# Arief-AK/OpenCL-Development-Real-time-Image-Processing

Measured on AMD Instinct MI355X. Metric: Mpixels/s (Gaussian 5x5, 4K RGBA), higher is better.
Workload: dtype u8 in/out, f32 accumulate

## Files before the change

### opencl-development-real-time-image-processing_amd/csrc/capi.hip

```cpp
#include <hip/hip_runtime.h>

#include <cmath>
#include <cstdio>
#include <cstdlib>
#include <cstring>
#include <ctime>
#include <new>
#include <vector>

#include "../../include/mi355_imgfilter.h"
#include "kernels.hpp"

using namespace mi355;

namespace {

struct CoefEntry {
    int k;
    uint32_t sigma_bits;
    GaussCoef coef;
    float* d_buf;
    std::vector<float> h_tab;
    uint64_t last_use;
    bool installed;
};

constexpr size_t kMaxCoefEntries = 16;
constexpr size_t kMaxInstalledCoefs = 64;

struct DevBuf {
    void* p;
    size_t cap;
};

}

struct mi355_ctx {
    int device = 0;
    hipStream_t stream = nullptr;
    bool own_stream = false;
    hipEvent_t ev[6] = {};
    hipEvent_t t0 = nullptr, t1 = nullptr;
    DevBuf d_in = {}, d_out = {};
    DevBuf d_raw = {};
    DevBuf d_flags = {};
    DevBuf d_hist = {};
    DevBuf d_lut = {};
    DevBuf d_ccl = {};
    DevBuf d_map1 = {}, d_map2 = {};
    unsigned long long* d_acc = nullptr;
    float* d_img_table = nullptr;
    static constexpr int kSlots = 3;
    hipStream_t s_h2d = nullptr, s_d2h = nullptr;
    hipEvent_t ev_h2d[kSlots] = {}, ev_k[kSlots] = {}, ev_d2h[kSlots] = {};
    DevBuf slot_in[kSlots] = {}, slot_out[kSlots] = {}, slot_raw[kSlots] = {};
    int input_format = MI355_INPUT_RGBA;
    int gauss_mode = MI355_GAUSS_FAST;
    int impl = MI355_IMPL_AUTO;
    int last_hip = 0;
    char name[256] = {};
    std::vector<CoefEntry> coefs;
    uint64_t coef_clock = 0;
    std::vector<void*> pinned;
};

namespace {

#define HIP_TRY(ctx, expr)                     \
    do {                                       \
        hipError_t e__ = (expr);               \
        if (e__ != hipSuccess) {               \
            if (ctx)                           \
                (ctx)->last_hip = (int)e__;    \
            return MI355_ERR_HIP;              \
        }                                      \
    } while (0)

uint64_t now_ns()
{
    timespec ts;
    clock_gettime(CLOCK_MONOTONIC, &ts);
    return (uint64_t)ts.tv_sec * 1000000000ull + (uint64_t)ts.tv_nsec;
}

uint32_t fbits(float f)
{
    uint32_t u;
    std::memcpy(&u, &f, 4);
    return u;
}

bool valid_k(int k) { return k >= 1 && k <= MI355_MAX_GAUSS_K && (k & 1) == 1; }
bool valid_sigma(float s) { return std::isfinite(s) && s > 0.0f; }

void gen_weights(int k, float sigma, float* out)
{
    const int half = k / 2;
    float sum = 0.0f;
    for (int y = -half; y <= half; y++) {
        for (int x = -half; x <= half; x++) {
            const float arg = -(x * x + y * y) / (2 * sigma * sigma);
            const float value = (float)(std::exp((double)arg) / (2 * M_PI * sigma * sigma));
            out[(y + half) * k + (x + half)] = value;
            sum += value;
        }
    }
    for (int i = 0; i < k * k; i++)
        out[i] /= sum;
}

void gen_weights_image2d(int k, float sigma, float* out)
{
    const int half = k / 2;
    for (int i = 0; i < k * k; i++)
        out[i] = 0.0f;
    float sum = 0.0f;
    for (int x = -half; x < half; x++) {
        for (int y = -half; y < half; y++) {
            const float arg = -((x * x + y * y) / (2 * sigma * sigma));
            const float value = (float)(std::exp((double)arg) / (2 * M_PI * sigma * sigma));
            out[(x + half) * k + (y + half)] = value;
// ... 7 lines not shown
bool separable_factor(int k, const float* w2d, float* w1d)
{
    double tot = 0.0, wmax = 0.0;
    bool nonneg = true;
    std::vector<double> rs(k, 0.0);
    for (int i = 0; i < k; i++) {
        for (int j = 0; j < k; j++) {
            const double v = (double)w2d[i * k + j];
            rs[i] += v;
            nonneg = nonneg && v >= 0.0;
            wmax = std::fmax(wmax, std::fabs(v));
        }
        tot += rs[i];
    }
    if (!nonneg || !(tot > 0.0)) {
        for (int i = 0; i < k; i++)
            w1d[i] = 0.0f;
        return false;
    }
    const double s = std::sqrt(tot);
    for (int i = 0; i < k; i++)
        w1d[i] = (float)(rs[i] / s);
    double dev = 0.0;
    for (int i = 0; i < k; i++)
        for (int j = 0; j < k; j++)
            dev = std::fmax(dev, std::fabs((double)w2d[i * k + j] - (double)w1d[i] * (double)w1d[j]));
    return dev <= 1.0e-6 * wmax;
}

int install_coef(mi355_ctx* ctx, int k, float sigma, const float* w2d, bool installed, const GaussCoef** out)
{
    CoefEntry* slot = nullptr;
    size_t n_generated = 0, n_installed = 0;
    for (auto& e : ctx->coefs) {
        if (e.k == k && e.sigma_bits == fbits(sigma))
            slot = &e;
        (e.installed ? n_installed : n_generated)++;
    }
    if (!slot) {
        if (installed && n_installed >= kMaxInstalledCoefs)
            return MI355_ERR_BAD_ARG;
        if (!installed && n_generated >= kMaxCoefEntries) {
            HIP_TRY(ctx, hipStreamSynchronize(ctx->stream));
            size_t lru = ctx->coefs.size();
            for (size_t i = 0; i < ctx->coefs.size(); i++)
                if (!ctx->coefs[i].installed && (lru == ctx->coefs.size() || ctx->coefs[i].last_use < ctx->coefs[lru].last_use))
                    lru = i;
            (void)hipFree(ctx->coefs[lru].d_buf);
            ctx->coefs.erase(ctx->coefs.begin() + (long)lru);
        }
        CoefEntry e{};
        e.k = k;
        e.sigma_bits = fbits(sigma);
        HIP_TRY(ctx, hipMalloc((void**)&e.d_buf, sizeof(float) * (size_t)(k * k + k + 512)));
        ctx->coefs.push_back(e);
        slot = &ctx->coefs.back();
    }
    slot->last_use = ++ctx->coef_clock;
    slot->installed = slot->installed || installed;
    std::vector<float> host((size_t)k * k + k + 512);
    std::memcpy(host.data(), w2d, sizeof(float) * (size_t)k * k);
    const bool separable = separable_factor(k, w2d, host.data() + (size_t)k * k);
    uint32_t alpha_tab[256];
    for (uint32_t a = 0; a < 256; a++)
        alpha_tab[a] = gauss_const_alpha(host.data() + (size_t)k * k, k, a) << 24;
    std::memcpy(host.data() + (size_t)k * k + k, alpha_tab, sizeof(alpha_tab));
    uint32_t alpha_cpu[256];
    for (uint32_t a = 0; a < 256; a++) {
        float chain = 0.0f;
        for (int i = 0; i < k * k; i++)
            chain += (float)a * w2d[i];
        chain = chain < 0.0f ? 0.0f : (chain > 255.0f ? 255.0f : chain);
        alpha_cpu[a] = (uint32_t)chain << 16;
    }
    std::memcpy(host.data() + (size_t)k * k + k + 256, alpha_cpu, sizeof(alpha_cpu));
    const hipError_t ce = hipMemcpy(slot->d_buf, host.data(), sizeof(float) * host.size(), hipMemcpyHostToDevice);
    if (ce != hipSuccess) {
        ctx->last_hip = (int)ce;
        (void)hipFree(slot->d_buf);
        ctx->coefs.erase(ctx->coefs.begin() + (slot - ctx->coefs.data()));
        return MI355_ERR_HIP;
    }
    slot->coef.k = k;
    slot->coef.separable = separable;
    slot->coef.d_w2d = slot->d_buf;
    slot->coef.d_w1d = slot->d_buf + (size_t)k * k;
    slot->coef.d_alpha_tab = reinterpret_cast<const uint32_t*>(slot->d_buf + (size_t)k * k + k);
    std::memcpy(slot->coef.h_alpha_tab, alpha_tab, sizeof(alpha_tab));
    slot->coef.d_alpha_cpu = reinterpret_cast<const uint32_t*>(slot->d_buf + (size_t)k * k + k + 256);
    std::memcpy(slot->coef.h_alpha_cpu, alpha_cpu, sizeof(alpha_cpu));
    std::memset(slot->coef.h_w1d, 0, sizeof(slot->coef.h_w1d));
    std::memcpy(slot->coef.h_w1d, host.data() + (size_t)k * k, sizeof(float) * k);
    slot->h_tab = host;
    slot->coef.h_w2d = slot->h_tab.data();
    if (out)
        *out = &slot->coef;
    return MI355_OK;
}

int get_coef(mi355_ctx* ctx, int k, float sigma, const GaussCoef** out)
{
    for (auto& e : ctx->coefs)
        if (e.k == k && e.sigma_bits == fbits(sigma)) {
            e.last_use = ++ctx->coef_clock;
            *out = &e.coef;
            return MI355_OK;
        }
    std::vector<float> w((size_t)k * k);
    gen_weights(k, sigma, w.data());
    return install_coef(ctx, k, sigma, w.data(), false, out);
}

int ensure(mi355_ctx* ctx, DevBuf& b, size_t need)
{
    if (b.cap >= need)
        return MI355_OK;
    if (b.p) {
        HIP_TRY(ctx, hipStreamSynchronize(ctx->stream));
        HIP_TRY(ctx, hipFree(b.p));
        b = {};
    }
    size_t want = need + need / 4;
    hipError_t e = hipMalloc(&b.p, want);
    if (e != hipSuccess) {
        e = hipMalloc(&b.p, need);
        want = need;
    }
    if (e != hipSuccess) {
        ctx->last_hip = (int)e;
        b.p = nullptr;
        return MI355_ERR_NOMEM;
    }
    b.cap = want;
    return MI355_OK;
}

int ensure_slots(mi355_ctx* ctx, DevBuf (&slots)[mi355_ctx::kSlots], size_t need)
{
    if (slots[0].cap >= need)
        return MI355_OK;
    HIP_TRY(ctx, hipDeviceSynchronize());
    for (DevBuf& b : slots) {
        if (b.p)
            (void)hipFree(b.p);
        b = {};
    }
    for (DevBuf& b : slots)
        if (hipMalloc(&b.p, need) != hipSuccess)
            return MI355_ERR_NOMEM;
    for (DevBuf& b : slots)
        b.cap = need;
    return MI355_OK;
}

enum class KRule { none, gauss, median, morph, box };

struct FilterInfo {
    int id;
    int in_bpp, out_bpp;
    KRule k;
    bool table;
    bool below_2g;
};

constexpr FilterInfo kFilters[] = {
    {MI355_FILTER_GRAY, 4, 4, KRule::none, false, false},
// ... 337 lines not shown
    if (!(rx < limit) || !(ry < limit))
        return MI355_ERR_UNSUPPORTED;
    if (inv)
        for (int k = 0; k < 6; k++)
            inv[k] = i[k];
    return MI355_OK;
}

int check_two_shapes(int bpp, int src_w, int src_h, int dst_w, int dst_h, int nframes, int border_mode)
{
    if (bad_shapes(bpp, src_w, src_h, dst_w, dst_h, nframes, border_mode))
        return MI355_ERR_BAD_ARG;
    const int rc = check_shape_limits(src_w, src_h, dst_w, dst_h, nframes);
    if (rc == MI355_OK && remap_work_items(dst_w, dst_h, nframes) > 0x7FFFFFF0ull)
        return MI355_ERR_BAD_ARG;
    return rc;
}

void map_bytes(int dst_w, int dst_h, int map_kind, size_t* n1, size_t* n2)
{
    const size_t entries = (size_t)dst_w * dst_h;
    *n1 = entries * 4;
    *n2 = entries * (map_kind == MI355_MAP_FIXED ? 2 : 4);
}

void perspective_inverse(const double m[9], int flags, double inv[9])
{
    if (flags & MI355_WARP_INVERSE_MAP) {
        for (int i = 0; i < 9; i++)
            inv[i] = m[i];
        return;
    }
    const double det = m[0] * (m[4] * m[8] - m[5] * m[7]) - m[1] * (m[3] * m[8] - m[5] * m[6]) +
                       m[2] * (m[3] * m[7] - m[4] * m[6]);
    const double d = (det != 0.0) ? 1.0 / det : 0.0;
    inv[0] = (m[4] * m[8] - m[5] * m[7]) * d;
    inv[1] = (m[2] * m[7] - m[1] * m[8]) * d;
    inv[2] = (m[1] * m[5] - m[2] * m[4]) * d;
    inv[3] = (m[5] * m[6] - m[3] * m[8]) * d;
    inv[4] = (m[0] * m[8] - m[2] * m[6]) * d;
    inv[5] = (m[2] * m[3] - m[0] * m[5]) * d;
    inv[6] = (m[3] * m[7] - m[4] * m[6]) * d;
    inv[7] = (m[1] * m[6] - m[0] * m[7]) * d;
    inv[8] = (m[0] * m[4] - m[1] * m[3]) * d;
}

int check_perspective(int bpp, int src_w, int src_h, int dst_w, int dst_h, int nframes, const double* m, int flags,
                      int border_mode, double* inv)
{
    if (!m || !warp_flags_ok(flags) || bad_shapes(bpp, src_w, src_h, dst_w, dst_h, nframes, border_mode) ||
        !all_finite(m, 9))
        return MI355_ERR_BAD_ARG;
    const int rc = check_two_shapes(bpp, src_w, src_h, dst_w, dst_h, nframes, border_mode);
    if (rc == MI355_OK && inv)
        perspective_inverse(m, flags, inv);
    return rc;
}

int adaptive_idelta(int type, double delta)
{
    const double d = type == MI355_ADAPTIVE_BINARY ? std::ceil(delta) : std::floor(delta);
    return d < -256.0 ? -256 : (d > 256.0 ? 256 : (int)d);
}

int create_common(int device, hipStream_t stream, bool own, mi355_ctx** out)
{
    if (!out)
        return MI355_ERR_BAD_ARG;
    *out = nullptr;
    int n = 0;
    if (hipGetDeviceCount(&n) != hipSuccess || n <= 0)
        return MI355_ERR_NO_DEVICE;
    if (device < 0 || device >= n)
        return MI355_ERR_NO_DEVICE;
    hipDeviceProp_t prop;
    if (hipGetDeviceProperties(&prop, device) != hipSuccess)
        return MI355_ERR_NO_DEVICE;
    if (std::strncmp(prop.gcnArchName, "gfx950", 6) != 0)
        return MI355_ERR_UNSUPPORTED;
    mi355_ctx* ctx = new (std::nothrow) mi355_ctx();
    if (!ctx)
        return MI355_ERR_NOMEM;
    ctx->device = device;
    std::snprintf(ctx->name, sizeof(ctx->name), "%s (%s)", prop.name, prop.gcnArchName);
    bool ok = hipSetDevice(device) == hipSuccess;
    if (ok && own)
        ok = hipStreamCreateWithFlags(&stream, hipStreamNonBlocking) == hipSuccess;
    ctx->stream = stream;
    ctx->own_stream = own && ok;
    for (int i = 0; ok && i < 6; i++)
        ok = hipEventCreate(&ctx->ev[i]) == hipSuccess;
    ok = ok && hipEventCreate(&ctx->t0) == hipSuccess && hipEventCreate(&ctx->t1) == hipSuccess;
    ok = ok && hipMalloc((void**)&ctx->d_acc, sizeof(unsigned long long)) == hipSuccess;
    if (!ok) {
        mi355_ctx_destroy(ctx);
        return MI355_ERR_HIP;
    }
    *out = ctx;
    return MI355_OK;
}

}

extern "C" {

#define MI355_API __attribute__((visibility("default")))

MI355_API int mi355_device_count(int* count)
{
    if (!count)
        return MI355_ERR_BAD_ARG;
    int n = 0;
    if (hipGetDeviceCount(&n) != hipSuccess)
        n = 0;
    *count = n;
    return MI355_OK;
}

MI355_API int mi355_ctx_create(int device, mi355_ctx** out)
{
    return create_common(device, nullptr, true, out);
}

MI355_API int mi355_ctx_create_on_stream(int device, void* hip_stream, mi355_ctx** out)
{
    return create_common(device, static_cast<hipStream_t>(hip_stream), false, out);
}

MI355_API int mi355_ctx_destroy(mi355_ctx* ctx)
{
    if (!ctx)
        return MI355_ERR_BAD_ARG;
    (void)hipSetDevice(ctx->device);
    (void)hipStreamSynchronize(ctx->stream);
    for (auto& e : ctx->coefs)
        (void)hipFree(e.d_buf);
    for (void* p : ctx->pinned)
        (void)hipHostFree(p);
    for (void* p : {(void*)ctx->d_acc, (void*)ctx->d_img_table, ctx->d_in.p, ctx->d_out.p, ctx->d_raw.p, ctx->d_flags.p,
                    ctx->d_hist.p, ctx->d_lut.p, ctx->d_ccl.p, ctx->d_map1.p, ctx->d_map2.p})
        if (p)
            (void)hipFree(p);
    for (int i = 0; i < mi355_ctx::kSlots; i++) {
        for (void* p : {ctx->slot_in[i].p, ctx->slot_out[i].p, ctx->slot_raw[i].p})
            if (p)
                (void)hipFree(p);
        for (hipEvent_t ev : {ctx->ev_h2d[i], ctx->ev_k[i], ctx->ev_d2h[i]})
            if (ev)
                (void)hipEventDestroy(ev);
    }
    for (hipStream_t s : {ctx->s_h2d, ctx->s_d2h})
        if (s)
            (void)hipStreamDestroy(s);
    for (hipEvent_t ev : {ctx->ev[0], ctx->ev[1], ctx->ev[2], ctx->ev[3], ctx->ev[4], ctx->ev[5], ctx->t0, ctx->t1})
        if (ev)
            (void)hipEventDestroy(ev);
    if (ctx->own_stream && ctx->stream)
        (void)hipStreamDestroy(ctx->stream);
    delete ctx;
    return MI355_OK;
}

MI355_API int mi355_ctx_device_name(mi355_ctx* ctx, char* buf, size_t buflen)
{
    if (!ctx || !buf || buflen == 0)
        return MI355_ERR_BAD_ARG;
// ... 1234 lines not shown
```

### opencl-development-real-time-image-processing_amd/csrc/common.hpp

```cpp
#pragma once
#include <hip/hip_runtime.h>
#include <stdint.h>

#include <cstdlib>
#include <type_traits>
#include <utility>

namespace mi355 {

constexpr int kWave = 64;

template <int... Ks, typename F>
hipError_t dispatch_int(int v, std::integer_sequence<int, Ks...>, F&& f)
{
    hipError_t e = hipErrorInvalidValue;
    (void)((v == Ks && ((e = f(std::integral_constant<int, Ks>{})), true)) || ...);
    return e;
}

template <typename F>
hipError_t dispatch_bool(bool v, F&& f)
{
    return v ? f(std::true_type{}) : f(std::false_type{});
}

inline bool aligned_to(const void* p, size_t n)
{
    return (reinterpret_cast<uintptr_t>(p) & (n - 1)) == 0;
}

inline bool rows_ragged(int w, const void* d_in, size_t in_align, const void* d_out, size_t out_align)
{
    return (w & 3) != 0 || !aligned_to(d_in, in_align) || !aligned_to(d_out, out_align);
}

inline bool gauss_upper_clamp(double wsum, double slack = 0.0)
{
    return !(255.0 * wsum * wsum * 1.0001 + slack < 256.0);
}

inline const char* tune_env(const char* name)
{
#ifdef MI355_TUNE_ENV
    return getenv(name);
#else
    (void)name;
    return nullptr;
#endif
}

using u32x4 = __attribute__((ext_vector_type(4))) uint32_t;
using u32x2 = __attribute__((ext_vector_type(2))) uint32_t;
using f32x4 = __attribute__((ext_vector_type(4))) float;

__device__ __forceinline__ uint32_t luma_rgb(uint32_t r, uint32_t g, uint32_t b)
{
    double v = 0.299 * (double)r + 0.587 * (double)g + 0.114 * (double)b;
    return (uint32_t)v;
}

__device__ __forceinline__ uint32_t luma_px(uint32_t px)
{
    return luma_rgb(px & 0xFFu, (px >> 8) & 0xFFu, (px >> 16) & 0xFFu);
}

__device__ __forceinline__ float luma_px_fast(uint32_t px)
{
    const uint32_t hi = __builtin_amdgcn_udot4(px, 0x00000201u, 0u, false);
    const uint32_t lo = __builtin_amdgcn_udot4(px, 0x00724B2Bu, 0u, false);
    const float S = (float)((hi << 8) + lo);
    float q = __builtin_floorf(__builtin_fmaf(S, 0.001f, 0.0005f));
    if (__builtin_fmaf(q, -1000.0f, S) == 0.0f)
        q = (float)luma_px(px);
    return q;
}

__device__ __forceinline__ void fill_gray_lut(uint8_t* gray_lut)
{
    gray_lut[threadIdx.x] = (uint8_t)luma_rgb(threadIdx.x, threadIdx.x, threadIdx.x);
}

__device__ __forceinline__ uint32_t luma_px_ambiguous(uint32_t px, const uint8_t* gray_lut)
{
    if (((px ^ (px >> 8)) & 0xFFFFu) == 0u)
        return gray_lut[px & 0xFFu];
    return luma_px(px);
}

__device__ __forceinline__ void luma_quad_fast(const u32x4& p, float g[4])
{
    float rem[4];
#pragma unroll
    for (int j = 0; j < 4; j++) {
        const uint32_t hi = __builtin_amdgcn_udot4(p[j], 0x00000201u, 0u, false);
        const uint32_t lo = __builtin_amdgcn_udot4(p[j], 0x00724B2Bu, 0u, false);
        const float S = (float)((hi << 8) + lo);
        g[j] = __builtin_floorf(__builtin_fmaf(S, 0.001f, 0.0005f));
        rem[j] = __builtin_fmaf(g[j], -1000.0f, S);
    }
    if (fminf(fminf(rem[0], rem[1]), fminf(rem[2], rem[3])) == 0.0f) {
#pragma unroll
        for (int j = 0; j < 4; j++)
            if (rem[j] == 0.0f)
                g[j] = (float)luma_px(p[j]);
    }
}

__device__ __forceinline__ bool gray_row(const u32x4& p, float g[4], const uint8_t* gray_lut)
{
    const uint32_t ng = ((p.x ^ (p.x >> 8)) | (p.y ^ (p.y >> 8)) | (p.z ^ (p.z >> 8)) | (p.w ^ (p.w >> 8))) & 0xFFFFu;
    if (__builtin_amdgcn_ballot_w64(ng != 0u) != 0)
        return false;
#pragma unroll
    for (int j = 0; j < 4; j++)
        g[j] = (float)gray_lut[p[j] & 0xFFu];
    return true;
}

__device__ __forceinline__ void luma_quad_fast(const u32x4& p, float g[4], const uint8_t* gray_lut, bool& gray_run)
{
    if (gray_run) {
        if (gray_row(p, g, gray_lut))
            return;
        gray_run = false;
    }
    float rem[4];
#pragma unroll
    for (int j = 0; j < 4; j++) {
        const uint32_t hi = __builtin_amdgcn_udot4(p[j], 0x00000201u, 0u, false);
        const uint32_t lo = __builtin_amdgcn_udot4(p[j], 0x00724B2Bu, 0u, false);
        const float S = (float)((hi << 8) + lo);
        g[j] = __builtin_floorf(__builtin_fmaf(S, 0.001f, 0.0005f));
// ... 173 lines not shown
```

### opencl-development-real-time-image-processing_amd/csrc/gauss_slide.hip

```cpp
#include <cmath>
#include <cstdlib>
#include <type_traits>

#include "common.hpp"
#include "kernels.hpp"
#include "slide_common.hpp"

namespace mi355 {

namespace {

constexpr uint32_t kRowStoreNowhere = 0x80000000u;
__device__ __forceinline__ void gstore_row_nt(global_ptr<uint8_t> rowp, uint32_t row_bytes, uint32_t off, u32x4 v)
{
    const auto rsrc = __builtin_amdgcn_make_buffer_rsrc((void*)rowp, (short)0, (int)row_bytes, 0x00020000);
    __builtin_amdgcn_raw_buffer_store_b128(v, rsrc, (int)off, 0, 2 );
}

constexpr uint32_t kSlideLdsForFiveWaves = 160u * 1024u / 5u - 1024u;
template <typename... KArgs, typename... Args>
hipError_t launch_slide_lds(void (*kernel)(KArgs...), const BandPlan& plan, uint32_t lds_bytes, hipStream_t stream,
                            Args... args)
{
    hipLaunchKernelGGL(kernel, dim3(plan.nblocks_a + plan.nblocks_b), dim3(kSlideWavesPerBlock * 64), lds_bytes, stream,
// ... 72 lines not shown
    return (uint32_t)a;
}

template <bool CLAMP>
__device__ __forceinline__ uint32_t pack_px(float a, float b, float c, float d)
{
    if constexpr (CLAMP) {
        a = fminf(a, 255.0f);
        b = fminf(b, 255.0f);
        c = fminf(c, 255.0f);
        d = fminf(d, 255.0f);
    }
    return (uint32_t)a | ((uint32_t)b << 8) | ((uint32_t)c << 16) | ((uint32_t)d << 24);
}

__device__ __forceinline__ void hpass5_dpp(float v0, float v1, float v2, float v3, float w0, float w1, float w2,
                                           float w3, float w4, float& o0, float& o1, float& o2, float& o3)
{
    asm volatile(
        "s_nop 1\n\t"
        "v_mul_f32_dpp %0, %6, %8 wave_shr:1 row_mask:0xf bank_mask:0xf bound_ctrl:1\n\t"
        "v_mul_f32_dpp %1, %7, %8 wave_shr:1 row_mask:0xf bank_mask:0xf bound_ctrl:1\n\t"
        "v_mul_f32_e32 %2, %8, %4\n\t"
        "v_mul_f32_e32 %3, %8, %5\n\t"
        "v_fmac_f32_dpp %0, %7, %9 wave_shr:1 row_mask:0xf bank_mask:0xf bound_ctrl:1\n\t"
        "v_fmac_f32_e32 %1, %9, %4\n\t"
        "v_fmac_f32_e32 %2, %9, %5\n\t"
        "v_fmac_f32_e32 %3, %9, %6\n\t"
        "v_fmac_f32_e32 %0, %10, %4\n\t"
        "v_fmac_f32_e32 %1, %10, %5\n\t"
        "v_fmac_f32_e32 %2, %10, %6\n\t"
        "v_fmac_f32_e32 %3, %10, %7\n\t"
        "v_fmac_f32_e32 %0, %11, %5\n\t"
        "v_fmac_f32_e32 %1, %11, %6\n\t"
        "v_fmac_f32_e32 %2, %11, %7\n\t"
        "v_fmac_f32_dpp %3, %4, %11 wave_shl:1 row_mask:0xf bank_mask:0xf bound_ctrl:1\n\t"
        "v_fmac_f32_e32 %0, %12, %6\n\t"
        "v_fmac_f32_e32 %1, %12, %7\n\t"
        "v_fmac_f32_dpp %2, %4, %12 wave_shl:1 row_mask:0xf bank_mask:0xf bound_ctrl:1\n\t"
        "v_fmac_f32_dpp %3, %5, %12 wave_shl:1 row_mask:0xf bank_mask:0xf bound_ctrl:1"
        : "=&v"(o0), "=&v"(o1), "=&v"(o2), "=&v"(o3)
        : "v"(v0), "v"(v1), "v"(v2), "v"(v3), "v"(w0), "v"(w1), "v"(w2), "v"(w3), "v"(w4));
}

struct SlideLane {
    global_ptr<const uint8_t> fin;
    global_ptr<uint8_t> fout;
    size_t row_bytes;
    SlideGeom g;
    int y0, nout, h;
    uint32_t px_off[4];
    int w;
    RaggedEdge edge;
};

template <bool NA0>
__device__ __forceinline__ bool alpha_row_differs(const u32x4& p, uint32_t nA)
{
    uint32_t t;
    if constexpr (NA0)
        t = (p.x & p.y) & (p.z & p.w);
    else
        t = ((p.x ^ nA) & (p.y ^ nA)) & ((p.z ^ nA) & (p.w ^ nA));
    return __builtin_amdgcn_ballot_w64(t < 0xFF000000u) != 0;
}

constexpr int kBandDone = 0;
constexpr int kBandAbortUniform = 1;
constexpr int kBandAbort = 2;
constexpr int kBandAbortUniformFirst = 3;

template <typename F, int... I>
__device__ __forceinline__ void static_rows_impl(F&& f, std::integer_sequence<int, I...>)
{
    (f(std::integral_constant<int, I>{}), ...);
}
template <int N, typename F>
__device__ __forceinline__ void static_rows(F&& f)
{
    static_rows_impl(f, std::make_integer_sequence<int, N>{});
}


template <int R, bool CLAMP, int NCH, bool RAGGED, bool UP, int AMODE, bool LOCKSTEP>
__device__ __forceinline__ int gauss_slide_band(const SlideLane& L, const float (&wv)[2 * R + 1], uint32_t alpha_hi,
                                                const uint32_t* __restrict__ alpha_tab, u32x4 (&q3)[2 * R + 1],
                                                bool preloaded)
{
    constexpr int K = 2 * R + 1;
    static_assert((NCH == 4) == (AMODE == 0), "AMODE 1 / 2 belong to the 3-channel pass");
    uint32_t in_off = L.g.in_off, out_off = L.g.out_off;
    [[maybe_unused]] const uint32_t out_voff = L.g.stores ? out_off : kRowStoreNowhere;
    const BandWalk W = band_walk(UP, L.y0, L.nout, R, L.h);
    uint32_t cur_nA = 0u;
    int run = 0;
    int code = kBandDone;
    const ptrdiff_t step_bytes = UP ? -(ptrdiff_t)L.row_bytes : (ptrdiff_t)L.row_bytes;
    const int y_lo = max(L.y0 - R, 0), y_hi = min(L.y0 + L.nout - 1 + R, L.h - 1);
    int y_in = W.y_first;
    auto in_p = L.fin + (size_t)clampi(y_in, y_lo, y_hi) * L.row_bytes;
    auto out_p = L.fout + (size_t)out_row(W, 0) * L.row_bytes;
    auto next_in_row = [&]() {
        const int y_next = y_in + W.y_step;
        in_p += (min(y_in, y_next) >= y_lo && max(y_in, y_next) <= y_hi) ? step_bytes : (ptrdiff_t)0;
        y_in = y_next;
    };
    auto load_row = [&]() -> u32x4 {
        const auto rowp = in_p;
        next_in_row();
        if constexpr (R <= 2)
            lane_offset_here(in_off);
        if constexpr (RAGGED) {
            if (L.w < 4) {
                u32x4 r;
#pragma unroll
                for (int j = 0; j < 4; j++)
                    r[j] = gload<uint32_t>(rowp + L.px_off[j]);
                return r;
            }
            return gload_a4<u32x4>(rowp + in_off);
        } else {
            return gload<u32x4>(rowp + in_off);
        }
    };

    constexpr int PF = (K < 3) ? K : 3;
    u32x4 q_own[K];
    u32x4 (&q)[K] = (AMODE == 0) ? q_own : q3;
    if (AMODE != 2 || !preloaded) {
#pragma unroll
        for (int u = 0; u < PF; u++)
            q[u] = load_row();
    } else {
#pragma unroll
        for (int u = 0; u < PF; u++)
            next_in_row();
    }
    if constexpr (AMODE == 1) {
        if (alpha_row_differs<true>(q[0], 0u)) {
            const uint32_t a_row = ((uint32_t)__builtin_amdgcn_readfirstlane((int)q[0].x) >> 24) & 0xFFu;
            return alpha_row_differs<false>(q[0], (a_row ^ 0xFFu) << 24) ? kBandAbort : kBandAbortUniformFirst;
        }
    }

    constexpr bool kRing = R <= 3;
    static_assert(kRing || !UP, "the accumulator form walks down only");
    float rows[K][4 * NCH] = {};

    auto do_row = [&](auto slot, auto outputs) __attribute__((always_inline)) {
        constexpr int u = decltype(slot)::value;
        constexpr bool OUT = decltype(outputs)::value;
        {
            u32x4 p_copy = q[u];
            u32x4& p = *((PF < K) ? &q[u] : &p_copy);
            if constexpr (LOCKSTEP) {
                __builtin_amdgcn_s_barrier();
            }
            if constexpr (PF < K)
                q[(u + PF) % K] = load_row();
            if (L.g.edge_strip) {
                if constexpr (!RAGGED) {
                    if (L.g.left_of_image)
                        p = u32x4{p.x, p.x, p.x, p.x};
                    if (L.g.right_of_image)
                        p = u32x4{p.w, p.w, p.w, p.w};
                } else if (L.w >= 4) {
                    if (L.g.left_of_image)
                        p = u32x4{p.x, p.x, p.x, p.x};
                    ragged_shift_clamp(p, L.edge);
                }
            }
            if constexpr (AMODE == 1) {
                if (alpha_row_differs<true>(p, 0u) && code == kBandDone) {
                    const uint32_t a_row = ((uint32_t)__builtin_amdgcn_readfirstlane((int)p.x) >> 24) & 0xFFu;
                    code = alpha_row_differs<false>(p, (a_row ^ 0xFFu) << 24) ? kBandAbort : kBandAbortUniform;
                }
            }
            if constexpr (AMODE == 2) {
                if (alpha_row_differs<false>(p, cur_nA)) {
                    const uint32_t a_new = ((uint32_t)__builtin_amdgcn_readfirstlane((int)p.x) >> 24) & 0xFFu;
                    const uint32_t nA = (a_new ^ 0xFFu) << 24;
                    if (alpha_row_differs<false>(p, nA))
                        code = kBandAbort;
                    cur_nA = nA;
                    alpha_hi = __builtin_amdgcn_readfirstlane(alpha_tab[a_new]);
                    run = 0;
                }
                run++;
            }
            if constexpr (kRing) {
#pragma unroll
                for (int px = 0; px < 4; px++)
#pragma unroll
                    for (int c = 0; c < NCH; c++)
                        rows[u][px * NCH + c] = ubyte_f32(p[px], c);
            } else {
#pragma unroll
                for (int px = 0; px < 4; px++) {
                    float f[NCH];
#pragma unroll
                    for (int c = 0; c < NCH; c++)
                        f[c] = ubyte_f32(p[px], c);
#pragma unroll
                    for (int j = 0; j < K; j++) {
                        const int sl = (u - j + K) % K;
#pragma unroll
                        for (int c = 0; c < NCH; c++)
                            rows[sl][px * NCH + c] =
                                (j == 0) ? wv[0] * f[c] : __builtin_fmaf(wv[j], f[c], rows[sl][px * NCH + c]);
// ... 34 lines not shown
                        cvt_pack3x4(hres, alpha_hi, o);
                    }
                } else {
                    float v[4 * NCH];
#pragma unroll
                    for (int e = 0; e < 4 * NCH; e++)
                        v[e] = vsum(e);
#pragma unroll
                    for (int px = 0; px < 4; px++) {
                        float r4[4] = {0.0f, 0.0f, 0.0f, 0.0f};
#pragma unroll
                        for (int c = 0; c < NCH; c++) {
                            float sum = 0.0f;
#pragma unroll
                            for (int t = 0; t < K; t++) {
                                const int s = px - R + t;
                                float src;
                                if (s < 0)
                                    src = dpp_left(v[(4 + s) * NCH + c]);
                                else if (s > 3)
                                    src = dpp_right(v[(s - 4) * NCH + c]);
                                else
                                    src = v[s * NCH + c];
                                sum = (t == 0) ? wv[0] * src : __builtin_fmaf(wv[t], src, sum);
                            }
                            r4[c] = sum;
                        }
                        o[px] = pack_px<CLAMP>(r4[0], r4[1], r4[2], r4[3]);
                        if constexpr (NCH == 3)
                            o[px] |= alpha_hi;
                    }
                }
                const auto rowp = out_p;
                out_p += step_bytes;
                if constexpr (!RAGGED) {
                    gstore_row_nt(rowp, (uint32_t)L.row_bytes, out_voff, o);
                } else if (L.g.stores) {
                    if constexpr (R <= 2)
                        lane_offset_here(out_off);
                    if constexpr (RAGGED) {
                        if (L.g.edge_strip && L.g.x_lane + 3 >= L.w) {
#pragma unroll
                            for (int j = 0; j < 4; j++)
                                if (L.g.x_lane + j < L.w)
                                    gstore_a4<uint32_t>(rowp + out_off + 4 * j, o[j]);
                        } else {
                            gstore_a4<u32x4>(rowp + out_off, o);
                        }
                    } else {
                        gstore_nt<u32x4>(rowp + out_off, o);
                    }
                }
            }
        }
    };
    static_rows<2 * R>([&](auto v) __attribute__((always_inline)) { do_row(v, std::false_type{}); });
    const int ntrips = L.nout / K, rem = L.nout - ntrips * K;
    auto trip = [&]() __attribute__((always_inline)) {
        static_rows<K>([&](auto v) __attribute__((always_inline)) {
            do_row(std::integral_constant<int, (2 * R + decltype(v)::value) % K>{}, std::true_type{});
        });
    };
    constexpr int kPeeled = RAGGED ? 0 : 1;
    if (ntrips >= kPeeled) {
        if constexpr (kPeeled)
            trip();
        for (int t = kPeeled; t < ntrips && code == kBandDone; t++)
            trip();
    }
    auto rem_rows = [&](auto self, auto v) __attribute__((always_inline)) {
        constexpr int V = decltype(v)::value;
        if constexpr (V < K - 1) {
            if (V < rem) {
                do_row(std::integral_constant<int, (2 * R + V) % K>{}, std::true_type{});
                self(self, std::integral_constant<int, V + 1>{});
            }
        }
    };
    if (code == kBandDone)
        rem_rows(rem_rows, std::integral_constant<int, 0>{});
    return code;
}

template <int R, bool CLAMP, bool RAGGED, int MODE, bool LOCKSTEP>
__global__ __launch_bounds__(kSlideWavesPerBlock * 64, (R == 3 && MODE == 3) ? 3 : 1) void gauss_slide_kernel(
    const uint8_t* __restrict__ in, uint8_t* __restrict__ out, int w, int h, int nstrips, int lanes_out,
    BandPlan plan, Weights<2 * R + 1> wts, uint32_t alpha_hi, const uint32_t* __restrict__ alpha_tab,
    uint32_t* __restrict__ flags)
{
    constexpr int K = 2 * R + 1;
    const int lane = threadIdx.x & 63;
    SlideItem it;
    if (!slide_item(plan, nstrips, h, &it))
        return;
    if constexpr (MODE == 4) {
        if (flags[it.work] == 0)
            return;
    }
    SlideLane L;
    L.g = slide_geom<4>(it.strip, lanes_out, lane, w, 16u, 16u);
    L.y0 = it.y0;
    L.nout = it.nout;
    L.h = h;
    L.w = w;
    L.row_bytes = (size_t)w * 4;
    L.fin = uniform_ptr(in + it.frame * L.row_bytes * h);
    L.fout = uniform_ptr(out + it.frame * L.row_bytes * h);
    L.edge = RaggedEdge{false, false, false, false};
    if constexpr (RAGGED) {
        if (w >= 4)
            L.g.in_off = ragged_edge_setup(L.g.q_lane, L.g.q_load, w, &L.edge);
    }
#pragma unroll
    for (int j = 0; j < 4; j++)
        L.px_off[j] = (uint32_t)clampi(L.g.x_lane + j, 0, w - 1) * 4u;

    float wv[K];
#pragma unroll
    for (int j = 0; j < K; j++) {
        wv[j] = wts.w[j];
        asm volatile("" : "+v"(wv[j]));
    }

    const bool up = (it.band & 1) != 0;
    u32x4 q3[K];
    auto run = [&](auto amode, bool preloaded) -> int {
        constexpr int AMODE = decltype(amode)::value;
        constexpr int NCH = AMODE == 0 ? 4 : 3;
        if constexpr (R <= 3) {
            if (up)
                return gauss_slide_band<R, CLAMP, NCH, RAGGED, true, AMODE, LOCKSTEP>(L, wv, alpha_hi, alpha_tab, q3, preloaded);
        }
        return gauss_slide_band<R, CLAMP, NCH, RAGGED, false, AMODE, LOCKSTEP>(L, wv, alpha_hi, alpha_tab, q3, preloaded);
    };
    auto three_channels = [&]() -> int {
        int code = run(std::integral_constant<int, 1>{}, false);
        if (code == kBandAbortUniform || code == kBandAbortUniformFirst)
            code = run(std::integral_constant<int, 2>{}, code == kBandAbortUniformFirst);
        return code;
    };
    if constexpr (MODE == 0) {
        if (three_channels() != kBandDone)
            run(std::integral_constant<int, 0>{}, false);
    } else if constexpr (MODE == 3) {
        const int code = three_channels();
        if (lane == 0)
            flags[it.work] = code == kBandDone ? 0u : 1u;
    } else {
        run(std::integral_constant<int, 0>{}, false);
    }
}

template <int R>
bool slide_plan(int w, int h, int nframes, bool ragged, StripPlan* sp, BandPlan* plan)
{
    constexpr int K = 2 * R + 1;
    *sp = make_strip_plan(w);
    if (K == 5) {
        const bool big = (size_t)sp->nstrips * ((h + 23) / 24) * nframes >= 2800;
        const int rows = (big && !ragged) ? 15 : 24;
        return make_band_plan(h, sp->nstrips, nframes, 4, rows, rows, rows, 0.0, 12, plan);
    }
    return (K == 3)   ? make_band_plan(h, sp->nstrips, nframes, 5, 12, 12, 12, 0.0, 6, plan)
                      : make_band_plan(h, sp->nstrips, nframes, 3, 96, 270, 40, 0.1, 4 * R + 4, plan);
}

template <int R>
hipError_t launch_r(hipStream_t stream, const uint8_t* d_in, uint8_t* d_out, int w, int h, int nframes,
                    const GaussCoef& coef, uint32_t* d_flags)
{
    constexpr int K = 2 * R + 1;
    constexpr bool kSplit = R >= 3;
    StripPlan sp;
    BandPlan plan;
    const bool ragged = rows_ragged(w, d_in, 16, d_out, 16) || (size_t)w * 4 > kRowStoreNowhere;
    if (!slide_plan<R>(w, h, nframes, ragged, &sp, &plan) || (kSplit && !d_flags))
        return hipErrorInvalidValue;
    const int nstrips = sp.nstrips, lanes_out = sp.lanes_out;
    Weights<K> wts;
    for (int j = 0; j < K; j++)
        wts.w[j] = coef.h_w1d[j];
    double wsum = 0.0;
    for (int j = 0; j < K; j++)
        wsum += (double)coef.h_w1d[j];
    if (!coef.d_alpha_tab)
        return hipErrorInvalidValue;
    const uint32_t alpha_hi = coef.h_alpha_tab[255];
    const uint32_t* alpha_tab = coef.d_alpha_tab;
    const bool lockstep =
        R <= 2 && !ragged && nstrips % kSlideWavesPerBlock == 0 && plan.nwork_b == 0 && plan.nwork_a >= 8192u;
    const uint32_t lds_bytes = (R == 1 && !ragged) ? kSlideLdsForFiveWaves : 0u;
    auto launch = [&](auto kernel) {
        return launch_slide_lds(kernel, plan, lds_bytes, stream, d_in, d_out, w, h, nstrips, lanes_out, plan, wts, alpha_hi,
                                alpha_tab, d_flags);
    };
    return dispatch_bool(gauss_upper_clamp(wsum), [&](auto CL) {
        return dispatch_bool(ragged, [&](auto RG) {
            if constexpr (kSplit) {
                const hipError_t e = launch(gauss_slide_kernel<R, CL.value, RG.value, 3, false>);
                return e != hipSuccess ? e : launch(gauss_slide_kernel<R, CL.value, RG.value, 4, false>);
            } else if constexpr (RG.value) {
                return launch(gauss_slide_kernel<R, CL.value, true, 0, false>);
            } else {
                return dispatch_bool(
                    lockstep, [&](auto LS) { return launch(gauss_slide_kernel<R, CL.value, false, 0, LS.value>); });
            }
        });
    });
}

}

bool gauss_slide_supported(const uint8_t* d_in, const uint8_t* d_out, int w, int h, int k)
{
    (void)h;
    (void)w;
    if (k != 3 && k != 5 && k != 7 && k != 9)
        return false;
    return aligned_to(d_in, 4) && aligned_to(d_out, 4);
}

size_t gauss_slide_flag_items(int w, int h, int nframes, int k)
{
    StripPlan sp;
    BandPlan plan;
    const hipError_t e = dispatch_int(k, std::integer_sequence<int, 7, 9>{}, [&](auto K) {
        return slide_plan<K.value / 2>(w, h, nframes, false, &sp, &plan) ? hipSuccess : hipErrorInvalidValue;
    });
    return e == hipSuccess ? (size_t)plan.nwork_a + plan.nwork_b : 0;
}

hipError_t launch_gauss_slide(hipStream_t stream, const uint8_t* d_in, uint8_t* d_out, int w, int h,
                              int nframes, const GaussCoef& coef, uint32_t* d_flags)
{
    return dispatch_int(coef.k, std::integer_sequence<int, 3, 5, 7, 9>{}, [&](auto K) {
        return launch_r<K.value / 2>(stream, d_in, d_out, w, h, nframes, coef, d_flags);
    });
}

}
```

### opencl-development-real-time-image-processing_amd/csrc/kernels.hpp

```cpp
#pragma once
#include <hip/hip_runtime.h>
#include <stdint.h>

namespace mi355 {

struct GaussCoef {
    int k;
    const float* d_w2d;
    const float* d_w1d;
    float h_w1d[64];
    const float* h_w2d;
    bool separable;
    const uint32_t* d_alpha_tab;
    uint32_t h_alpha_tab[256];
    const uint32_t* d_alpha_cpu;
    uint32_t h_alpha_cpu[256];
};

uint32_t gauss_const_alpha(const float* w1d, int k, uint32_t a);

hipError_t launch_gray(hipStream_t stream, const uint8_t* d_in, uint8_t* d_out, int w, int h,
                       int nframes, bool one_channel);

size_t gauss_flag_items(const uint8_t* d_in, const uint8_t* d_out, int w, int h, int nframes, const GaussCoef& coef,
                        bool exact, int impl);
hipError_t launch_gauss(hipStream_t stream, const uint8_t* d_in, uint8_t* d_out, int w, int h,
                        int nframes, const GaussCoef& coef, bool exact, int impl, uint32_t* d_flags);

hipError_t launch_gauss_tile(hipStream_t stream, const uint8_t* d_in, uint8_t* d_out, int w, int h,
                             int nframes, const GaussCoef& coef, bool exact);

bool gauss_slide_supported(const uint8_t* d_in, const uint8_t* d_out, int w, int h, int k);
size_t gauss_slide_flag_items(int w, int h, int nframes, int k);
hipError_t launch_gauss_slide(hipStream_t stream, const uint8_t* d_in, uint8_t* d_out, int w, int h,
                              int nframes, const GaussCoef& coef, uint32_t* d_flags);

bool gauss_wide_supported(const uint8_t* d_in, const uint8_t* d_out, int w, int h, int k);
size_t gauss_wide_flag_items(int w, int h, int nframes, int k);
hipError_t launch_gauss_wide(hipStream_t stream, const uint8_t* d_in, uint8_t* d_out, int w, int h, int nframes,
                             const GaussCoef& coef, uint32_t* d_flags);

bool gauss_exact_supported(const uint8_t* d_in, const uint8_t* d_out, int w, int h, const GaussCoef& coef);
hipError_t launch_gauss_exact(hipStream_t stream, const uint8_t* d_in, uint8_t* d_out, int w, int h, int nframes,
                              const GaussCoef& coef);

bool gauss_mfma_reg_supported(const uint8_t* d_in, const uint8_t* d_out, int w, int h, const GaussCoef& coef);
hipError_t launch_gauss_mfma_reg(hipStream_t stream, const uint8_t* d_in, uint8_t* d_out, int w, int h, int nframes,
                                 const GaussCoef& coef);

hipError_t launch_sobel(hipStream_t stream, const uint8_t* d_in, uint8_t* d_out, int w, int h,
                        int nframes, int impl);
bool sobel_slide_supported(const uint8_t* d_in, const uint8_t* d_out, int w, int h);
hipError_t launch_sobel_slide(hipStream_t stream, const uint8_t* d_in, uint8_t* d_out, int w, int h, int nframes);

hipError_t launch_pipeline(hipStream_t stream, const uint8_t* d_in, uint8_t* d_out, int w, int h,
                           int nframes, const GaussCoef& coef, bool exact, int impl);
bool pipe_slide_supported(const uint8_t* d_in, const uint8_t* d_out, int w, int h, const GaussCoef& coef, int px);
hipError_t launch_pipe_slide(hipStream_t stream, const uint8_t* d_in, uint8_t* d_out, int w, int h, int nframes,
                             const GaussCoef& coef, int px);

hipError_t launch_gauss_gray8(hipStream_t stream, const uint8_t* d_in, uint8_t* d_out, int w, int h, int nframes,
                              const GaussCoef& coef, bool exact, int impl);
hipError_t launch_sobel_gray8(hipStream_t stream, const uint8_t* d_in, uint8_t* d_out, int w, int h, int nframes);
hipError_t launch_pipeline_gray8(hipStream_t stream, const uint8_t* d_in, uint8_t* d_out, int w, int h, int nframes,
                                 const GaussCoef& coef, int impl);

hipError_t launch_median(hipStream_t stream, const uint8_t* d_in, uint8_t* d_out, int w, int h, int nframes, int k,
                         bool gray8, int impl);

hipError_t launch_morph(hipStream_t stream, const uint8_t* d_in, uint8_t* d_out, int w, int h, int nframes, int k,
                        int op, bool gray8);

hipError_t launch_hist(hipStream_t stream, const uint8_t* d_in, uint32_t* d_hist, int w, int h, int nframes);
hipError_t launch_hist_table(hipStream_t stream, const uint32_t* d_hist, uint8_t* d_lut, int32_t* d_thresh, int w,
                             int h, int nframes, bool otsu);
hipError_t launch_lut_apply(hipStream_t stream, const uint8_t* d_in, uint8_t* d_out, const uint8_t* d_lut, int w, int h,
                            int nframes);

constexpr int kClaheMaxTiles = 16;
struct ClaheGeom {
    int w, h, tiles_x, tiles_y;
    int tw, th;
    int cl;
    float lut_scale, inv_tw, inv_th;
};
hipError_t launch_clahe_hist(hipStream_t stream, const uint8_t* d_in, uint32_t* d_hist, const ClaheGeom& g, int nframes);
hipError_t launch_clahe_table(hipStream_t stream, const uint32_t* d_hist, uint8_t* d_luts, const ClaheGeom& g,
                              int nframes);
hipError_t launch_clahe_apply(hipStream_t stream, const uint8_t* d_in, uint8_t* d_out, const uint8_t* d_luts,
                              const ClaheGeom& g, int nframes);
// ... 73 lines not shown
```

### opencl-development-real-time-image-processing_amd/csrc/slide_common.hpp

```cpp
#pragma once
#include <cstdint>
#include <cstdlib>

#include "common.hpp"

namespace mi355 {

constexpr int kSlideLanesOutMax = 62;
constexpr int kSlideWavesPerBlock = 4;

struct BandPlan {
    int rows_a, nbands_a, rows_b, nbands_b, y_split;
    uint32_t nwork_a, nwork_b, nblocks_a, nblocks_b;
};

struct StripPlan {
    int quads, nstrips, lanes_out;
};

inline StripPlan make_strip_plan(int w, int lanes_pref = 0)
{
    StripPlan s;
    s.quads = (w + 3) / 4;
    s.nstrips = (s.quads + kSlideLanesOutMax - 1) / kSlideLanesOutMax;
    s.lanes_out = (s.quads + s.nstrips - 1) / s.nstrips;
    if (lanes_pref > 0 && lanes_pref <= kSlideLanesOutMax && s.nstrips > 1) {
        s.lanes_out = lanes_pref;
        s.nstrips = (s.quads + lanes_pref - 1) / lanes_pref;
    }
    static const int tune_lanes = [] {
        const char* e = tune_env("MI355_TUNE_LANES_OUT");
        return e ? atoi(e) : 0;
    }();
    if (tune_lanes > 0 && tune_lanes <= kSlideLanesOutMax) {
        s.lanes_out = tune_lanes;
        s.nstrips = (s.quads + tune_lanes - 1) / tune_lanes;
    }
    return s;
}

inline bool make_band_plan(int h, int nstrips, int nframes, int waves_per_simd, int rows_min, int rows_max,
                           int rows_tail, double tail_frac, int rows_small, BandPlan* out)
{
    const double resident = 256.0 * 4.0 * waves_per_simd;
    double rows = (double)h * nstrips * nframes / (10.0 * resident);
    int rows_big = (int)(rows < rows_min ? rows_min : (rows > rows_max ? rows_max : rows));
    static const struct Tune {
        int band_rows = 0, tail_rows = 0;
        double tail_frac = -1.0;
        Tune()
        {
            if (const char* e = tune_env("MI355_TUNE_BAND_ROWS"))
                band_rows = atoi(e);
            if (const char* e = tune_env("MI355_TUNE_TAIL_ROWS"))
                tail_rows = atoi(e);
            if (const char* e = tune_env("MI355_TUNE_TAIL_FRAC"))
                tail_frac = atof(e);
        }
    } tune;
    while (rows_small > 0 && rows_big / 2 >= rows_small &&
           (size_t)nstrips * ((h + rows_big - 1) / rows_big) * nframes < 2800)
        rows_big /= 2;
    if (tune.band_rows > 0)
        rows_big = tune.band_rows;
    if (tune.tail_rows > 0)
        rows_tail = tune.tail_rows;
    if (tune.tail_frac >= 0.0)
        tail_frac = tune.tail_frac;
    BandPlan p{};
    int h_b = (int)(h * tail_frac);
    if (h_b < rows_tail || h - h_b < rows_big || tail_frac <= 0.0 || rows_tail >= rows_big)
        h_b = 0;
    const int h_a = h - h_b;
    p.nbands_a = (h_a + rows_big - 1) / rows_big;
    p.rows_a = (h_a + p.nbands_a - 1) / p.nbands_a;
    p.y_split = h_a;
    if (h_b > 0) {
        p.nbands_b = (h_b + rows_tail - 1) / rows_tail;
        p.rows_b = (h_b + p.nbands_b - 1) / p.nbands_b;
    } else {
        p.nbands_b = 0;
        p.rows_b = 1;
    }
    const size_t na = (size_t)nstrips * p.nbands_a * nframes, nb = (size_t)nstrips * p.nbands_b * nframes;
    if (na + nb > 0x3FFFFFFFull)
        return false;
    p.nwork_a = (uint32_t)na;
    p.nwork_b = (uint32_t)nb;
    p.nblocks_a = (p.nwork_a + kSlideWavesPerBlock - 1) / kSlideWavesPerBlock;
    p.nblocks_b = (p.nwork_b + kSlideWavesPerBlock - 1) / kSlideWavesPerBlock;
    *out = p;
    return true;
}

#ifdef __HIPCC__
template <typename... KArgs, typename... Args>
hipError_t launch_slide(void (*kernel)(KArgs...), const BandPlan& plan, hipStream_t stream, Args... args)
{
    hipLaunchKernelGGL(kernel, dim3(plan.nblocks_a + plan.nblocks_b), dim3(kSlideWavesPerBlock * 64), 0, stream,
                       static_cast<KArgs>(args)...);
    return hipGetLastError();
}

template <typename T>
using global_ptr = __attribute__((address_space(1))) T*;

template <typename T>
__device__ __forceinline__ global_ptr<T> uniform_ptr(T* p)
{
    const uint64_t v = reinterpret_cast<uint64_t>(p);
    const uint32_t lo = __builtin_amdgcn_readfirstlane((uint32_t)v);
    const uint32_t hi = __builtin_amdgcn_readfirstlane((uint32_t)(v >> 32));
    return (global_ptr<T>)(((uint64_t)hi << 32) | lo);
}

__device__ __forceinline__ void lane_offset_here(uint32_t& off)
{
    asm volatile("" : "+v"(off));
}

template <typename V>
__device__ __forceinline__ V gload(global_ptr<const uint8_t> p)
{
    return *(global_ptr<const V>)p;
}
template <typename V>
__device__ __forceinline__ V gload_a4(global_ptr<const uint8_t> p)
{
    typedef V __attribute__((aligned(4))) VA;
    return *(global_ptr<const VA>)p;
}
template <typename V>
__device__ __forceinline__ void gstore_nt(global_ptr<uint8_t> p, V v)
{
    __builtin_nontemporal_store(v, (global_ptr<V>)p);
}
template <typename V>
__device__ __forceinline__ void gstore_a4(global_ptr<uint8_t> p, V v)
{
    typedef V __attribute__((aligned(4))) VA;
    *(global_ptr<VA>)p = v;
}

template <typename V>
__device__ __forceinline__ void gstore_a1(global_ptr<uint8_t> p, V v)
{
    typedef V __attribute__((aligned(1))) VA;
    *(global_ptr<VA>)p = v;
}

struct RaggedEdge {
    bool sh1, sh2, sh3, sh4;
};

__device__ __forceinline__ uint32_t ragged_edge_setup(int q_lane, int q_load, int w, RaggedEdge* e)
{
    const int xs = min(4 * q_load, w - 4);
    const int shift = 4 * q_lane - xs;
    e->sh1 = shift >= 1;
    e->sh2 = shift >= 2;
    e->sh3 = shift >= 3;
    e->sh4 = shift >= 4;
    return (uint32_t)xs * 4u;
}

__device__ __forceinline__ void ragged_shift_clamp(u32x4& p, const RaggedEdge& e)
{
    p.x = e.sh3 ? p.w : (e.sh2 ? p.z : (e.sh1 ? p.y : p.x));
    p.y = e.sh2 ? p.w : (e.sh1 ? p.z : p.y);
    p.z = e.sh1 ? p.w : p.z;
}

struct SlideItem {
    int strip, band, y0, nout;
    uint32_t work;
    size_t frame;
};
// ... 120 lines not shown
```

Baseline: 776,800.

## Use one-trip short bands for small Gaussian 5x5 workloads based on CU count

Adds a band plan for the 5x5 sliding Gaussian in which each wave handles roughly K rows. It is selected when the total work items fit within the device's wave slots (CU count × 4 SIMDs × 4 waves), which improves occupancy on small images. The CU count is plumbed from device properties into GaussCoef. The prefetch depth becomes a template parameter, still set to 3. tune_env moves to its own header, and the new path can be disabled through an environment knob.

```diff
diff --git a/opencl-development-real-time-image-processing_amd/csrc/capi.hip b/opencl-development-real-time-image-processing_amd/csrc/capi.hip
--- a/opencl-development-real-time-image-processing_amd/csrc/capi.hip
+++ b/opencl-development-real-time-image-processing_amd/csrc/capi.hip
@@ -37,6 +37,7 @@
 
 struct mi355_ctx {
     int device = 0;
+    int cus = 0;
     hipStream_t stream = nullptr;
     bool own_stream = false;
     hipEvent_t ev[6] = {};
@@ -210,6 +211,7 @@
         return MI355_ERR_HIP;
     }
     slot->coef.k = k;
+    slot->coef.cus = ctx->cus;
     slot->coef.separable = separable;
     slot->coef.d_w2d = slot->d_buf;
     slot->coef.d_w1d = slot->d_buf + (size_t)k * k;
@@ -713,6 +715,7 @@
     if (!ctx)
         return MI355_ERR_NOMEM;
     ctx->device = device;
+    ctx->cus = prop.multiProcessorCount;
     std::snprintf(ctx->name, sizeof(ctx->name), "%s (%s)", prop.name, prop.gcnArchName);
     bool ok = hipSetDevice(device) == hipSuccess;
     if (ok && own)
diff --git a/opencl-development-real-time-image-processing_amd/csrc/common.hpp b/opencl-development-real-time-image-processing_amd/csrc/common.hpp
--- a/opencl-development-real-time-image-processing_amd/csrc/common.hpp
+++ b/opencl-development-real-time-image-processing_amd/csrc/common.hpp
@@ -6,6 +6,8 @@
 #include <type_traits>
 #include <utility>
 
+#include "tune_env.hpp"
+
 namespace mi355 {
 
 constexpr int kWave = 64;
@@ -39,15 +41,6 @@
     return !(255.0 * wsum * wsum * 1.0001 + slack < 256.0);
 }
 
-inline const char* tune_env(const char* name)
-{
-#ifdef MI355_TUNE_ENV
-    return getenv(name);
-#else
-    (void)name;
-    return nullptr;
-#endif
-}
 
 using u32x4 = __attribute__((ext_vector_type(4))) uint32_t;
 using u32x2 = __attribute__((ext_vector_type(2))) uint32_t;
diff --git a/opencl-development-real-time-image-processing_amd/csrc/gauss_slide.hip b/opencl-development-real-time-image-processing_amd/csrc/gauss_slide.hip
--- a/opencl-development-real-time-image-processing_amd/csrc/gauss_slide.hip
+++ b/opencl-development-real-time-image-processing_amd/csrc/gauss_slide.hip
@@ -178,7 +178,7 @@
 }
 
 
-template <int R, bool CLAMP, int NCH, bool RAGGED, bool UP, int AMODE, bool LOCKSTEP>
+template <int R, bool CLAMP, int NCH, bool RAGGED, bool UP, int AMODE, bool LOCKSTEP, int DEPTH>
 __device__ __forceinline__ int gauss_slide_band(const SlideLane& L, const float (&wv)[2 * R + 1], uint32_t alpha_hi,
                                                 const uint32_t* __restrict__ alpha_tab, u32x4 (&q3)[2 * R + 1],
                                                 bool preloaded)
@@ -220,7 +220,8 @@
         }
     };
 
-    constexpr int PF = (K < 3) ? K : 3;
+    static_assert(DEPTH >= 3 && DEPTH <= 4, "prefetch depths measured: 3 and 4");
+    constexpr int PF = (K < DEPTH) ? K : DEPTH;
     u32x4 q_own[K];
     u32x4 (&q)[K] = (AMODE == 0) ? q_own : q3;
     if (AMODE != 2 || !preloaded) {
@@ -421,6 +422,7 @@
     return code;
 }
 
+constexpr int kSlideRowsInFlight = 3;
 template <int R, bool CLAMP, bool RAGGED, int MODE, bool LOCKSTEP>
 __global__ __launch_bounds__(kSlideWavesPerBlock * 64, (R == 3 && MODE == 3) ? 3 : 1) void gauss_slide_kernel(
     const uint8_t* __restrict__ in, uint8_t* __restrict__ out, int w, int h, int nstrips, int lanes_out,
@@ -428,6 +430,7 @@
     uint32_t* __restrict__ flags)
 {
     constexpr int K = 2 * R + 1;
+    constexpr int kDepth = kSlideRowsInFlight;
     const int lane = threadIdx.x & 63;
     SlideItem it;
     if (!slide_item(plan, nstrips, h, &it))
@@ -468,9 +471,9 @@
         constexpr int NCH = AMODE == 0 ? 4 : 3;
         if constexpr (R <= 3) {
             if (up)
-                return gauss_slide_band<R, CLAMP, NCH, RAGGED, true, AMODE, LOCKSTEP>(L, wv, alpha_hi, alpha_tab, q3, preloaded);
+                return gauss_slide_band<R, CLAMP, NCH, RAGGED, true, AMODE, LOCKSTEP, kDepth>(L, wv, alpha_hi, alpha_tab, q3, preloaded);
         }
-        return gauss_slide_band<R, CLAMP, NCH, RAGGED, false, AMODE, LOCKSTEP>(L, wv, alpha_hi, alpha_tab, q3, preloaded);
+        return gauss_slide_band<R, CLAMP, NCH, RAGGED, false, AMODE, LOCKSTEP, kDepth>(L, wv, alpha_hi, alpha_tab, q3, preloaded);
     };
     auto three_channels = [&]() -> int {
         int code = run(std::integral_constant<int, 1>{}, false);
@@ -491,12 +494,18 @@
 }
 
 template <int R>
-bool slide_plan(int w, int h, int nframes, bool ragged, StripPlan* sp, BandPlan* plan)
+bool slide_plan(int w, int h, int nframes, bool ragged, int cus, StripPlan* sp, BandPlan* plan)
 {
     constexpr int K = 2 * R + 1;
     *sp = make_strip_plan(w);
     if (K == 5) {
+        static const bool one_trip_bands = [] {
+            const char* e = tune_env("MI355_TUNE_GAUSS_SMALL");
+            return !e || atoi(e) != 0;
+        }();
         const bool big = (size_t)sp->nstrips * ((h + 23) / 24) * nframes >= 2800;
+        if (!big && !ragged && one_trip_bands && one_trip_bands_leave_slots(h, sp->nstrips, nframes, K, cus, 4))
+            return make_one_trip_band_plan(h, sp->nstrips, nframes, K, 4, plan);
         const int rows = (big && !ragged) ? 15 : 24;
         return make_band_plan(h, sp->nstrips, nframes, 4, rows, rows, rows, 0.0, 12, plan);
     }
@@ -513,7 +522,7 @@
     StripPlan sp;
     BandPlan plan;
     const bool ragged = rows_ragged(w, d_in, 16, d_out, 16) || (size_t)w * 4 > kRowStoreNowhere;
-    if (!slide_plan<R>(w, h, nframes, ragged, &sp, &plan) || (kSplit && !d_flags))
+    if (!slide_plan<R>(w, h, nframes, ragged, coef.cus, &sp, &plan) || (kSplit && !d_flags))
         return hipErrorInvalidValue;
     const int nstrips = sp.nstrips, lanes_out = sp.lanes_out;
     Weights<K> wts;
@@ -564,7 +573,7 @@
     StripPlan sp;
     BandPlan plan;
     const hipError_t e = dispatch_int(k, std::integer_sequence<int, 7, 9>{}, [&](auto K) {
-        return slide_plan<K.value / 2>(w, h, nframes, false, &sp, &plan) ? hipSuccess : hipErrorInvalidValue;
+        return slide_plan<K.value / 2>(w, h, nframes, false, 0, &sp, &plan) ? hipSuccess : hipErrorInvalidValue;
     });
     return e == hipSuccess ? (size_t)plan.nwork_a + plan.nwork_b : 0;
 }
diff --git a/opencl-development-real-time-image-processing_amd/csrc/kernels.hpp b/opencl-development-real-time-image-processing_amd/csrc/kernels.hpp
--- a/opencl-development-real-time-image-processing_amd/csrc/kernels.hpp
+++ b/opencl-development-real-time-image-processing_amd/csrc/kernels.hpp
@@ -6,6 +6,7 @@
 
 struct GaussCoef {
     int k;
+    int cus;
     const float* d_w2d;
     const float* d_w1d;
     float h_w1d[64];
diff --git a/opencl-development-real-time-image-processing_amd/csrc/slide_common.hpp b/opencl-development-real-time-image-processing_amd/csrc/slide_common.hpp
--- a/opencl-development-real-time-image-processing_amd/csrc/slide_common.hpp
+++ b/opencl-development-real-time-image-processing_amd/csrc/slide_common.hpp
@@ -2,7 +2,11 @@
 #include <cstdint>
 #include <cstdlib>
 
+#ifdef __HIPCC__
 #include "common.hpp"
+#else
+#include "tune_env.hpp"
+#endif
 
 namespace mi355 {
 
@@ -93,6 +97,18 @@
     return true;
 }
 
+constexpr int kSimdsPerCu = 4;
+inline bool one_trip_bands_leave_slots(int h, int nstrips, int nframes, int K, int cus, int waves_per_simd)
+{
+    return (size_t)nstrips * ((h + K - 1) / K) * nframes <= (size_t)cus * kSimdsPerCu * waves_per_simd;
+}
+
+inline bool make_one_trip_band_plan(int h, int nstrips, int nframes, int K, int waves_per_simd, BandPlan* out)
+{
+    const int nbands = h >= K ? h / K : 1, rows = (h + nbands - 1) / nbands;
+    return make_band_plan(h, nstrips, nframes, waves_per_simd, rows, rows, rows, 0.0, 0, out);
+}
+
 #ifdef __HIPCC__
 template <typename... KArgs, typename... Args>
 hipError_t launch_slide(void (*kernel)(KArgs...), const BandPlan& plan, hipStream_t stream, Args... args)
diff --git a/opencl-development-real-time-image-processing_amd/csrc/tune_env.hpp b/opencl-development-real-time-image-processing_amd/csrc/tune_env.hpp
--- /dev/null
+++ b/opencl-development-real-time-image-processing_amd/csrc/tune_env.hpp
@@ -0,0 +1,16 @@
+#pragma once
+#include <cstdlib>
+
+namespace mi355 {
+
+inline const char* tune_env(const char* name)
+{
+#ifdef MI355_TUNE_ENV
+    return getenv(name);
+#else
+    (void)name;
+    return nullptr;
+#endif
+}
+
+}
```

Result: slower. 764,700 (-1.6%).
